# adaliaramon/LambdaGap

Hardware: AMD Instinct MI355X
Metric: boosting iters/sec + AUC, synthetic Higgs-shape 10M×28, 255 bins, 63 leaves (higher is better)
Workload: dtype fp32; 1 GPU; model=gbdt binary, 63 leaves, 255 bins, lr 0.1, global_batch=10000000, seq_len=28, parallelism=dp1, device=AMD GPU (gfx950:sramecc+:xnack-) [frontier engine]

## Files before the change

src/device/device_learner.hip:

```cpp
#include <hip/hip_runtime.h>

#include <algorithm>
#include <chrono>
#include <cmath>
#include <cstdio>
#include <cstdlib>
#include <cstring>
#include <fstream>
#include <map>
#include <memory>
#include <string>
#include <vector>

#include "device/grad_kernels.h"
#include "device/hip_common.h"
#include "device/leaf_kernels.h"
#include "device/metric_kernels.h"
#include "device/linear_kernels.h"
#include "device/runtime_internal.h"
#include "device/frontier.h"
#include "device/policy_scan.h"
#include "device/traverse_kernels.h"
#include "device/sample_kernels.h"
#include "device/engine_plan.h"
#include "device/seq_kernels.h"
#include "device/split_scan.h"
#include "device/tree_kernels.h"
#include "learner/forced_splits.h"
#include "learner/linear_solve.h"
#include "learner/parallel_tree_learner.h"
#include "learner/serial_tree_learner.h"
#include "lgap/common.h"
#include "lgap/device_api.h"
#include "lgap/network.h"
#include "lgap/objective.h"
#include "lgap/rank_math.h"
#include "lgap/metric.h"
#include "lgap/split_math.h"

namespace lgap {
namespace device {
namespace {

const char* KernelOverride(const char* key) {
  static const char* const kKeys[] = {"fhist_threads", "hist_lds_kb", "quant_lds32", "part_iters",
                                      "hist_il",       "nibble",      "quant_hist",  "scan_global",
                                      "scan_wave",     "oob_rows",    "select_merge"};
  constexpr int kNumKeys = static_cast<int>(sizeof(kKeys) / sizeof(kKeys[0]));
  thread_local std::string vals[kNumKeys];
  const char* e = std::getenv("LGAP_KERNEL");
  if (e == nullptr) return nullptr;
  const std::string s(e);
  const char* found = nullptr;
  for (size_t p = 0; p < s.size();) {
    size_t q = s.find(',', p);
    if (q == std::string::npos) q = s.size();
    const std::string item = s.substr(p, q - p);
    p = q + 1;
    if (item.empty()) continue;
    const size_t eq = item.find('=');
    const std::string k = item.substr(0, eq);
    int idx = -1;
    for (int i = 0; i < kNumKeys; ++i) idx = k == kKeys[i] ? i : idx;
    if (idx < 0) Log::Fatal("LGAP_KERNEL: unknown key '%s'", k.c_str());
    if (k == key) {
      vals[idx] = eq == std::string::npos ? "1" : item.substr(eq + 1);
      found = vals[idx].c_str();
    }
  }
  return found;
}


using namespace seq;

template <typename T>
class PinnedBuf {
 public:
  ~PinnedBuf() {
    if (p_) (void)hipHostFree(p_);
  }
  T* Get(size_t n) {
    if (n > n_) {
      if (p_) HIP_CHECK(hipHostFree(p_));
      HIP_CHECK(hipHostMalloc(reinterpret_cast<void**>(&p_), std::max<size_t>(n, 1) * sizeof(T), hipHostMallocDefault));
      n_ = n;
    }
    return p_;
  }

 private:
  T* p_ = nullptr;
  size_t n_ = 0;
};

class DeviceTreeLearner : public TreeLearner {
 public:
  DeviceTreeLearner(const Config* config, const std::string& learner_type, bool routed = false)
      : config_(config), learner_type_(learner_type), routed_(routed) {}

// ... 1555 lines not shown
      if (num_tiles_ > 256) Log::Fatal("frontier histograms: %d LDS tiles (at most 256)", num_tiles_);
    }
    if (ffeature_ || fowner_) {
      std::vector<uint8_t> own(F_, 0);
      std::vector<int> list;
      for (int f : h_own_feat_) {
        if (f >= 0) {
          own[f] = 1;
          list.push_back(f);
        }
      }
      ffowned_.Upload(own, stream_);
      fown_n_ = static_cast<int>(list.size());
      fown_list_.Resize(std::max<size_t>(1, list.size()));
      if (!list.empty()) fown_list_.Upload(list.data(), list.size(), stream_);
      ffpb_.Resize(static_cast<size_t>(P_) * 2 * K);
    }
    if (fowner_) {
      fown_b0_.Upload(h_bin_lo_, stream_);
      const size_t send = static_cast<size_t>(P_) * K * bbin_ * 2;
      if (facc_.size() < send) facc_.Resize(send);
      facc_.Zero(stream_);
      facc_recv_.Resize(static_cast<size_t>(K) * bbin_ * 2);
    }
    if (plan_.bynode_on_device) {
      bool filt = false;
      const std::vector<uint8_t> m = col_sampler_.ByNodeSampleModes(&fbyn_cnt_, &filt);
      fbyn_reset_ = filt ? 1 : 0;
      fbyn_mode_.Resize(m.size());
      fbyn_mode_.Upload(m.data(), m.size(), stream_);
    }
    if (fvoting_) {
      SplitParams sl = MakeArgs().sp;
      sl.min_data_in_leaf = config_->min_data_in_leaf / P_;
      sl.min_sum_hessian_in_leaf = config_->min_sum_hessian_in_leaf / P_;
      fsp_local_.Resize(1);
      fsp_local_.Upload(&sl, 1, stream_);
      flsum_loc_.Resize(C);
      fltot_.Resize(2 * K);
      fltot_.Zero(stream_);
      fvrec_.Resize(static_cast<size_t>(P_) * 2 * K * topk_);
      fvelect_.Resize(2 * K * static_cast<size_t>(topk_ + 1));
      fvrows_.Resize(2 * K * static_cast<size_t>(topk_) * 2 * max_bin_);
    }
    fpart_iters_ = part_iters_;
    fpart_tile_ = kPartThreads * fpart_iters_;
    ftile_cap_ = DivUp(N_, fpart_tile_) + fkmax_ + 1;
    ftile_pub_.Resize(ftile_cap_);
    ftile_pub_.Zero(stream_);
    for (int i = 3; i < kFrontierIdx; ++i) idx_[i].Resize(std::max(N_, 1));
    {
      const int per_cu = std::max(1, FrontierPartitionBlocksPerCU(fpart_iters_));
      fpart_grid_ = std::max(1, std::min(ftile_cap_, per_cu * num_cu_));
    }
    fscan_lds_ = FrontierScanLds(max_bin_, has_cat_ ? max_cat_bin_ : 1);
    FrontierSetLds(FrontierHistLds(), fscan_lds_, use_dp_, width_);
    fspec_cap_ = 0;
    fhist_threads_ = big_tiles_ || (num_tiles_ == 1 && N_ >= 4000000) ? 1024 : 512;
    if (const char* e = KernelOverride("fhist_threads")) fhist_threads_ = std::atoi(e) == 1024 ? 1024 : 512;
    fpolicy_ = 1;
    fspec_alpha_ = 1.0;
    const char* spec_env = std::getenv("LGAP_FRONTIER_SPEC");
    const std::string spec = spec_env != nullptr ? spec_env : "";
    fspec_fixed_ = spec != "adapt";
    if (!spec.empty() && spec != "adapt" && spec != "fixed") {
      char* end = nullptr;
      const double alpha = std::strtod(spec.c_str(), &end);
      if (end == spec.c_str() || *end != '\0') Log::Fatal("LGAP_FRONTIER_SPEC=%s: expected fixed|adapt|<alpha>", spec.c_str());
      fspec_alpha_ = std::max(0.01, std::min(4.0, alpha));
    }
    {
      stune_ = SpecTuner();
      const char* te = std::getenv("LGAP_SPEC_TUNE");
      const bool tune_small = te == nullptr || te[0] != '0';
      stune_.on = !plan_.distributed && (L_ >= 128 || tune_small) && !plan_.raw_cands && fnum_forced_ == 0 &&
                  spec.empty();
      if (L_ < 128 && te == nullptr) stune_.rest = 64;
    }
    if (std::getenv("LGAP_FSTAMPS")) {
      fstamps_.Resize(256 * 4 * kFStampSlots);
      fstamps_.Zero(stream_);
    }
    for (auto& kv : fgraphs_) (void)hipGraphExecDestroy(kv.second);
    fgraphs_.clear();
    if (fcont_) (void)hipGraphExecDestroy(fcont_);
    fcont_ = nullptr;
  }

  FArgs MakeFArgs() const {
    FArgs a;
    std::memset(&a, 0, sizeof(a));
    a.rowbins = rowbins_.get();
    a.colbins = colbins_.get();
    a.gh = gh_.get();
    for (int i = 0; i < kFrontierIdx; ++i) a.idx[i] = idx_[i].get();
    a.N = N_;
    a.stride_dw = tstride_dw_;
    a.width = width_;
    a.num_groups = G_;
    a.TB = TB_;
    a.F = F_;
    a.L = L_;
    a.C = fC_;
    a.kmax = fkmax_;
    a.gstart = gstart_.get();
    a.feat = feat_.get();
// ... 411 lines not shown
    *num_splits = hs->num_splits;
    *num_leaves = hs->num_leaves;
    bynode_draws_ = hs->byn;
    bynode_rng_ = hs->byn_rng;
    if (*num_splits > 0) std::memcpy(hr, fres_host_ + FrontierResultRecOffset(), sizeof(SplitRec) * *num_splits);
    std::memcpy(hrange, fres_host_ + FrontierResultRangeOffset(L_), sizeof(LeafRange) * *num_leaves);
    *hlo = hh->lout0;
    unsigned hbar[4];
    std::memcpy(hbar, hh->bar, sizeof(hbar));
    if (hbar[3] != 0u) {
      static const char* const kinds[kFXKinds] = {"histogram", "split candidates", "root sums", "self-test"};
      Log::Fatal("xGMI exchange (%s) timed out on rank %d after %.0f s: a peer stopped training",
                 kinds[std::min<unsigned>(hbar[3] - 1u, kFXKinds - 1)], rank_, XTimeoutSeconds());
    }
    if (plan_.distributed) {
      std::memcpy(fkused_hist_[fkused_trees_ % 4], hh->kused, sizeof(int) * kFrontierRoundCap);
      ++fkused_trees_;
    }
    if (fstamps_.size() && fstat_trees_ == 3) ReportFrontierStamps(hs->round);
    if (fstamps_.size() && fstat_trees_ % 10 == 0) {
      std::fprintf(stderr, "frontier: %d trees, %.2f rounds/tree, %.2f expansions/tree (%d leaves max), wasted rows %.1f%%, "
                   "alpha %.3f, all-reduced expansion slots/tree %.1f, pipelined rounds/tree %.2f\n", fstat_trees_,
                   static_cast<double>(fstat_rounds_) / fstat_trees_, static_cast<double>(fstat_spec_) / fstat_trees_, L_,
                   100.0 * fstat_waste_ / fstat_trees_, stune_.on ? stune_.lo : fspec_alpha_, fstat_ar_exps_ / fstat_trees_,
                   static_cast<double>(fstat_pipelined_) / fstat_trees_);
    }
  }

  void ReportFrontierStamps(int rounds) {
    std::vector<unsigned long long> h(fstamps_.size());
    fstamps_.Download(h.data(), h.size(), stream_);
    HIP_CHECK(hipStreamSynchronize(stream_));
    static const char* names[4] = {"partition", "hist", "scan", "select"};
    auto at = [&](int r, int k, int i) { return h[(static_cast<size_t>(r) * 4 + k) * kFStampSlots + i]; };
    for (int k = 0; k < 4; ++k) {
      double acc[kFStampSlots] = {0};
      int cnt = 0;
      for (int r = 0; r < std::min(rounds + 1, 256); ++r) {
        const unsigned long long s0 = at(r, k, 0);
        if (!s0) continue;
        ++cnt;
        for (int i = 1; i < kFStampSlots; ++i) {
          const unsigned long long v = at(r, k, i);
          if (v >= s0) acc[i] += (v - s0) * 0.01;
        }
      }
      if (!cnt) continue;
      std::string line;
      for (int i = 1; i < kFStampSlots; ++i) {
        if (acc[i] > 0) line += " t" + std::to_string(i) + "=" + common::FormatG(acc[i] / cnt);
      }
      std::fprintf(stderr, "fstamps %s (%d rounds, us from block-0 start; t7 = last block exit):%s\n", names[k], cnt,
                   line.c_str());
      if (at(0, k, 0)) {
        std::string root;
        for (int i = 1; i < kFStampSlots; ++i) {
          const unsigned long long v = at(0, k, i);
          if (v >= at(0, k, 0) && v) root += " t" + std::to_string(i) + "=" + common::FormatG((v - at(0, k, 0)) * 0.01);
        }
        std::fprintf(stderr, "fstamps %s root round:%s\n", names[k], root.c_str());
      }
    }
    double gap[4] = {0};
    int cnt = 0;
    for (int r = 1; r + 1 < std::min(rounds, 255); ++r) {
      const unsigned long long P = at(r, 0, 0), H = at(r, 1, 0), S = at(r, 2, 0), Q = at(r, 3, 0), P2 = at(r + 1, 0, 0);
      if (!P || !H || !S || !Q || !P2 || !(P < H && H < S && S < Q && Q < P2)) continue;
      gap[0] += (H - P) * 0.01;
      gap[1] += (S - H) * 0.01;
      gap[2] += (Q - S) * 0.01;
      gap[3] += (P2 - Q) * 0.01;
      ++cnt;
    }
    if (cnt) {
      std::fprintf(stderr, "fstamps chain (%d rounds, start to start, us): partition->hist %.2f hist->scan %.2f "
                   "scan->select %.2f select->partition %.2f\n", cnt, gap[0] / cnt, gap[1] / cnt, gap[2] / cnt, gap[3] / cnt);
    }
  }

  void SequentialGrow(int* num_splits, int* num_leaves, SplitRec* hr, LeafRange* hrange, double* hlo) {
    const bool collectives = plan_.owner_scan || plan_.voting;
    const bool use_graph = config_->device_use_graph && (!collectives || (DPGraphEnabled() && !HostStagedDP()));
    if (use_graph) {
      if (graph_exec_ && plan_.distributed && graph_comm_ != ActiveComm()) InvalidateGraph();
      if (!graph_exec_) CaptureGraph();
      HIP_CHECK(hipGraphLaunch(graph_exec_, stream_));
    } else {
      EnqueueTree();
    }
    Ctl* hc2 = pin_ctl_.Get(2);
    HIP_CHECK(hipMemcpyAsync(hc2, ctl_.get(), 2 * sizeof(Ctl), hipMemcpyDeviceToHost, stream_));
    HIP_CHECK(hipMemcpyAsync(hr, rec_.get(), sizeof(SplitRec) * (L_ - 1), hipMemcpyDeviceToHost, stream_));
    HIP_CHECK(hipMemcpyAsync(hrange, range_.get(), sizeof(LeafRange) * L_, hipMemcpyDeviceToHost, stream_));
    HIP_CHECK(hipMemcpyAsync(hlo, lout_.get(), sizeof(double), hipMemcpyDeviceToHost, stream_));
    unsigned* hbar = pin_bar_.Get(4);
    HIP_CHECK(hipMemcpyAsync(hbar, bar_.get(), 4 * sizeof(unsigned), hipMemcpyDeviceToHost, stream_));
    if (collectives && !HostStagedDP()) {
      static const double timeout_s = CommTimeoutSeconds(config_->time_out);
      WatchedStreamSync(stream_, timeout_s, "device tree growth (RCCL histogram reduce-scatter)");
    } else {
      HIP_CHECK(hipStreamSynchronize(stream_));
    }
    if (hbar[2] != 0u) Log::Fatal("k_partition: a wait on published tile counts timed out (blocks not co-resident?)");
    const Ctl* hc = hc2[1].num_splits > hc2[0].num_splits ? &hc2[1] : &hc2[0];
    bynode_draws_ = 1 + 2 * hc->scan_round;
    *num_splits = hc->num_splits;
    *num_leaves = hc->num_leaves;
  }

  std::string DeviceName() const override {
    if (!plan_.owner_scan && !plan_.voting) {
      if (!frontier_) return device_name_;
      if (plan_.mono_inter) return device_name_ + " [frontier engine, intermediate monotone walk + rescans]";
// ... 1749 lines not shown
```

src/device/frontier_kernels.hip:

```cpp
#include <hip/hip_runtime.h>

#include <algorithm>
#include <cstdint>

#include "device/frontier.h"
#include "device/hip_common.h"
#include "device/split_scan.h"
#include "lgap/split_math.h"

namespace lgap {
namespace device {
namespace {

constexpr int kFPartThreads = 256;
constexpr int kFScanThreads = 256;
constexpr int kFSelThreads = 1024;
#ifndef LGAP_FHIST_R
#define LGAP_FHIST_R 16
#endif

__device__ __forceinline__ int FRowAt(const FArgs& a, int buf, int pos) { return buf < 0 ? pos : a.idx[buf][pos]; }

__device__ __forceinline__ uint32_t FColBin(const FArgs& a, int g, int row) {
  const size_t o = static_cast<size_t>(g) * a.N + row;
// ... 1238 lines not shown
      if (lane == 0) {
        key->feature = out->feature;
        key->gain = SafeGain(*out);
        key->threshold = out->threshold;
        key->group = fi.group;
        key->offset = fi.offset;
        key->num_bin = fi.num_bin;
        key->mfb = fi.mfb;
        key->default_bin = fi.default_bin;
        key->missing = fi.missing;
        key->default_left = out->default_left;
        key->is_cat = fi.bin_type != 0 ? 1 : 0;
        key->pad0 = a.cegb_raw && out->feature >= 0 ? out->monotone_type : 0;
      }
      FWaveSync();
      const size_t q = (static_cast<size_t>(e) * 2 + sel) * F + f;
      for (int i = lane; i < kKeyWords + kInfoWords; i += 64) {
        if (i < kKeyWords) {
          reinterpret_cast<uint32_t*>(a.ckey + q)[i] = reinterpret_cast<const uint32_t*>(key)[i];
        } else {
          reinterpret_cast<uint32_t*>(a.cinfo + q)[i - kKeyWords] = reinterpret_cast<const uint32_t*>(out)[i - kKeyWords];
        }
      }
      FWaveSync();
    }
    FWaveSync();
  }
  FStampEnd(a, rnd, kFStampScan);
}


__device__ __forceinline__ void FPublish(unsigned long long* p, unsigned epoch, int v, bool incl) {
  const unsigned long long w = (static_cast<unsigned long long>(epoch) << 32) | (incl ? 0x80000000ull : 0ull) |
                               static_cast<unsigned>(v);
  __hip_atomic_store(p, w, __ATOMIC_RELAXED, __HIP_MEMORY_SCOPE_AGENT);
}

__device__ __forceinline__ bool FGoLeft(const FExp& x, const uint32_t* bits, uint32_t gb) {
  const uint32_t b = DecodeBin(x.offset, x.num_bin, x.mfb, gb);
  if (x.is_cat) {
    const uint32_t wd = b >> 5;
    return wd < static_cast<uint32_t>(kMaxCatWords) && ((bits[wd] >> (b & 31u)) & 1u);
  }
  if ((x.missing == 1 && b == static_cast<uint32_t>(x.default_bin)) ||
      (x.missing == 2 && b == static_cast<uint32_t>(x.num_bin - 1))) {
    return x.default_left != 0;
  }
  return b <= static_cast<uint32_t>(x.thr);
}

constexpr unsigned kLookbackSpins = 2048;

constexpr int kLookbackPer = 4;

struct FLookbackLds {
  int near, nmiss, list[256 * kLookbackPer], val[256 * kLookbackPer], red[4];
};

__device__ int FLookback(const FArgs& a, const FExp& x, const uint32_t* bits, int i, unsigned epoch, FLookbackLds* L) {
  const int t = threadIdx.x;
  const int nt = static_cast<int>(blockDim.x);
  constexpr int kInf = 0x7fffffff;
  int excl = 0;
  for (int hi = i; hi > x.tile0;) {
    const int lo = max(x.tile0, hi - kLookbackPer * nt);
    unsigned long long v[kLookbackPer];
    bool have[kLookbackPer];
    if (t == 0) {
      L->near = kInf;
      L->nmiss = 0;
    }
#pragma unroll
    for (int u = 0; u < kLookbackPer; ++u) {
      const int j = hi - 1 - (u * nt + t);
      v[u] = j >= lo ? __hip_atomic_load(&a.tile_pub[j], __ATOMIC_RELAXED, __HIP_MEMORY_SCOPE_AGENT) : 0ull;
    }
#pragma unroll
    for (int u = 0; u < kLookbackPer; ++u) {
      const int j = hi - 1 - (u * nt + t);
      have[u] = false;
      if (j < lo) continue;
      for (unsigned spins = 0; static_cast<unsigned>(v[u] >> 32) != epoch && spins < kLookbackSpins; ++spins) {
        __builtin_amdgcn_s_sleep(1);
        v[u] = __hip_atomic_load(&a.tile_pub[j], __ATOMIC_RELAXED, __HIP_MEMORY_SCOPE_AGENT);
      }
      have[u] = static_cast<unsigned>(v[u] >> 32) == epoch && !a.part_selfcount;
    }
    __syncthreads();
#pragma unroll
    for (int u = 0; u < kLookbackPer; ++u) {
      const int j = hi - 1 - (u * nt + t);
      if (j >= lo && !have[u]) L->list[atomicAdd(&L->nmiss, 1)] = j;
    }
    __syncthreads();
    const int nm = L->nmiss;
    if (nm > 0) {
      for (int m = 0; m < nm; ++m) {
        const int tile = L->list[m];
        const int p0 = (tile - x.tile0) * a.part_tile, p1 = min(x.count, p0 + a.part_tile);
        int cc = 0;
        for (int p = p0 + t; p < p1; p += nt) {
          const int row = FRowAt(a, x.src_buf, x.start + p);
          cc += FGoLeft(x, bits, FColBin(a, x.group, row)) ? 1 : 0;
        }
        cc = BlockSumInt(cc, L->red);
        if (t == 0) {
          L->val[hi - 1 - tile] = cc;
          FPublish(&a.tile_pub[tile], epoch, cc, false);
        }
      }
      __syncthreads();
#pragma unroll
      for (int u = 0; u < kLookbackPer; ++u) {
        const int j = hi - 1 - (u * nt + t);
        if (j >= lo && !have[u]) {
          v[u] = static_cast<unsigned long long>(static_cast<unsigned>(L->val[u * nt + t]));
          have[u] = true;
        }
      }
    }
#pragma unroll
    for (int u = 0; u < kLookbackPer; ++u) {
      if (have[u] && (v[u] & 0x80000000ull) != 0ull) atomicMin(&L->near, u * nt + t);
    }
    __syncthreads();
    const int near = L->near;
    int c = 0;
#pragma unroll
    for (int u = 0; u < kLookbackPer; ++u) {
      const int j = hi - 1 - (u * nt + t);
      if (j >= lo && u * nt + t <= near) c += static_cast<int>(v[u] & 0x7fffffffull);
    }
    excl += BlockSumInt(c, L->red);
    if (near != kInf) break;
    hi = lo;
  }
  return excl;
}

__device__ void FPostSplit(const FArgs& a, int e, const FExp& x, int lc) {
  const SplitInfo& bi = x.forced >= 0 ? a.fbest[x.parent] : a.best[x.parent];
  const double lsg = bi.left_sum_gradient, lsh = bi.left_sum_hessian;
  const double rsg = bi.right_sum_gradient, rsh = bi.right_sum_hessian;
  const double lo = bi.left_output, ro = bi.right_output;
  const int ilc = bi.left_count, irc = bi.right_count;
  const int8_t mono = bi.monotone_type;
  const int16_t ncat = bi.num_cat_threshold;
  const int feature = bi.feature;
  LeafBounds bl = a.bounds[x.parent];
  const int rc = x.count - lc;
  const int glc = a.distributed ? ilc : lc;
  const int grc = a.distributed ? irc : rc;
  const int l = x.left, r = x.left + 1;
  const int dep = x.depth + 1;
  FNode nl, nr;
  nl.buf = nr.buf = x.dst_buf;
  nl.start = x.start;
  nl.count = lc;
  nl.gcount = glc;
  nr.start = x.start + lc;
  nr.count = rc;
  nr.gcount = grc;
  nl.depth = nr.depth = dep;
  nl.parent = nr.parent = x.parent;
  nl.left = nr.left = -1;
  nl.fidx = x.forced >= 0 ? a.forced[x.forced].left : -1;
  nr.fidx = x.forced >= 0 ? a.forced[x.forced].right : -1;
  a.nodes[l] = nl;
  a.nodes[r] = nr;
  a.lsum[l] = make_double2(lsg, lsh);
  a.lsum[r] = make_double2(rsg, rsh);
  a.lout[l] = lo;
  a.lout[r] = ro;
  LeafBounds br = bl;
  if (a.use_monotone && ncat == 0 && a.mono_inter) {
    if (mono < 0) {
      bl.min = fmax(bl.min, ro);
      br.max = fmin(br.max, lo);
    } else if (mono > 0) {
      bl.max = fmin(bl.max, ro);
      br.min = fmax(br.min, lo);
    }
  } else if (a.use_monotone && ncat == 0) {
    const double mid = (lo + ro) / 2.0f;
    if (mono < 0) {
      bl.min = fmax(bl.min, mid);
      br.max = fmin(br.max, mid);
    } else if (mono > 0) {
      bl.max = fmin(bl.max, mid);
      br.min = fmax(br.min, mid);
    }
  }
  a.bounds[l] = bl;
  a.bounds[r] = br;
  if (a.ic) {
    for (int w = 0; w < a.ic_words; ++w) {
      const unsigned long long icm = a.ic[static_cast<size_t>(x.parent) * a.ic_words + w] &
                                     a.ic_feat[static_cast<size_t>(feature) * a.ic_words + w];
      a.ic[static_cast<size_t>(l) * a.ic_words + w] = icm;
      a.ic[static_cast<size_t>(r) * a.ic_words + w] = icm;
    }
  }
  const int md = a.sp.min_data_in_leaf;
  const bool forced_child = nl.fidx >= 0 || nr.fidx >= 0;
  const bool skip = x.last || (!forced_child && ((a.max_depth > 0 && dep >= a.max_depth) || (grc < md * 2 && glc < md * 2)));
  const bool left_smaller = glc < grc;
  FExp* xo = a.exps + e;
  xo->skip = skip ? 1 : 0;
  xo->smaller = left_smaller ? l : r;
  xo->larger = left_smaller ? r : l;
  xo->h_buf = x.dst_buf;
  xo->h_start = left_smaller ? x.start : x.start + lc;
  xo->h_count = left_smaller ? lc : rc;
}

template <int M>
__device__ __forceinline__ void BlockSumMulti(int* v, int* sh) {
  const int lane = threadIdx.x & 63, w = threadIdx.x >> 6;
#pragma unroll
  for (int m = 0; m < M; ++m) v[m] = WaveSum(v[m]);
  __syncthreads();
  if (lane == 0) {
#pragma unroll
    for (int m = 0; m < M; ++m) sh[m * 4 + w] = v[m];
  }
  __syncthreads();
#pragma unroll
  for (int m = 0; m < M; ++m) v[m] = sh[m * 4] + sh[m * 4 + 1] + sh[m * 4 + 2] + sh[m * 4 + 3];
}

template <int ITERS, int MAXT>
__global__ __launch_bounds__(kFPartThreads) __attribute__((amdgpu_waves_per_eu(ITERS == 8 ? 5 : 1))) void k_f_partition(FArgs a) {
  static_assert(kFPartThreads == 256, "4 waves per block");
  static_assert(MAXT * ITERS <= 32, "left / valid bits of a thread fit one word");
  constexpr int kTile = kFPartThreads * ITERS;
  __shared__ int s_t0[kFrontierKmax + 1];
  __shared__ FExp s_x[kFrontierKmax];
  __shared__ uint32_t s_bits[kFrontierKmax][kMaxCatWords];
  __shared__ int sh[MAXT * 4];
  __shared__ int s_wl[MAXT][ITERS][kFPartThreads / 64];
  __shared__ int s_wv[MAXT][ITERS][kFPartThreads / 64];
  __shared__ FLookbackLds s_lb;
  const FState* stp = a.st;
  if (stp->done) return;
  const int k = stp->k, T = stp->total_tiles;
  const unsigned epoch = stp->epoch;
  const int rnd = stp->round;
  FStamp(a, rnd, kFStampPart, 0);
  const int G = static_cast<int>(gridDim.x);
  const int t = threadIdx.x;
  if (static_cast<int>(blockIdx.x) * MAXT >= T) return;
  constexpr int kXWords = static_cast<int>(sizeof(FExp) / 4);
  for (int i = t; i < k * kXWords; i += blockDim.x) {
    reinterpret_cast<uint32_t*>(s_x)[i] = reinterpret_cast<const uint32_t*>(a.exps)[i];
  }
  for (int i = t; i < k * kMaxCatWords; i += blockDim.x) s_bits[i / kMaxCatWords][i % kMaxCatWords] = a.exp_bits[i];
  __syncthreads();
  if (t <= k) s_t0[t] = t < k ? s_x[t].tile0 : T;
  __syncthreads();
  auto find = [&](int tile) {
    int lo = 0, hi = k - 1;
    while (lo < hi) {
      const int mid = (lo + hi + 1) >> 1;
      if (s_t0[mid] <= tile) lo = mid;
      else hi = mid - 1;
    }
    return lo;
  };
  auto go_left = [&](int e, uint32_t gb) { return FGoLeft(s_x[e], s_bits[e], gb); };
  FStamp(a, rnd, kFStampPart, 1);
  const int lane = t & 63, w = t >> 6;
  const unsigned long long lt_mask = (lane == 0) ? 0ull : (~0ull >> (64 - lane));
  for (int bid = static_cast<int>(blockIdx.x) * MAXT; bid < T; bid += G * MAXT) {
    int ex[MAXT], rows[MAXT][ITERS];
    unsigned lbits = 0u, vbits = 0u;
#pragma unroll
    for (int j = 0; j < MAXT; ++j) {
      const int tile = bid + j;
      ex[j] = tile < T ? find(tile) : -1;
      const int e = ex[j] < 0 ? 0 : ex[j];
      const FExp& x = s_x[e];
      const int pos0 = (tile - x.tile0) * kTile + t;
#pragma unroll
      for (int i = 0; i < ITERS; ++i) {
        const int pos = pos0 + i * kFPartThreads;
        rows[j][i] = (ex[j] >= 0 && pos < x.count) ? FRowAt(a, x.src_buf, x.start + pos) : -1;
      }
    }
    int cnt[MAXT];
    {
      uint32_t gb[MAXT][ITERS];
#pragma unroll
      for (int j = 0; j < MAXT; ++j) {
        const int g = s_x[ex[j] < 0 ? 0 : ex[j]].group;
#pragma unroll
        for (int i = 0; i < ITERS; ++i) gb[j][i] = rows[j][i] >= 0 ? FColBin(a, g, rows[j][i]) : 0u;
      }
#pragma unroll
      for (int j = 0; j < MAXT; ++j) {
        cnt[j] = 0;
#pragma unroll
        for (int i = 0; i < ITERS; ++i) {
          const bool valid = rows[j][i] >= 0;
          const bool left = valid && go_left(ex[j], gb[j][i]);
          vbits |= (valid ? 1u : 0u) << (j * ITERS + i);
          lbits |= (left ? 1u : 0u) << (j * ITERS + i);
          cnt[j] += left ? 1 : 0;
        }
      }
    }
    BlockSumMulti<MAXT>(cnt, sh);
    if (t == 0) {
#pragma unroll
      for (int j = 0; j < MAXT; ++j) {
        if (ex[j] >= 0) FPublish(&a.tile_pub[bid + j], epoch, cnt[j], bid + j == s_x[ex[j]].tile0);
      }
    }
    FStamp(a, rnd, kFStampPart, 2);
    int lb[MAXT];
    lb[0] = ex[0] >= 0 && bid > s_x[ex[0]].tile0 ? FLookback(a, s_x[ex[0]], s_bits[ex[0]], bid, epoch, &s_lb) : 0;
#pragma unroll
    for (int j = 1; j < MAXT; ++j) lb[j] = ex[j] >= 0 && ex[j] == ex[j - 1] ? lb[j - 1] + cnt[j - 1] : 0;
    if (t == 0) {
#pragma unroll
      for (int j = 0; j < MAXT; ++j) {
        if (ex[j] >= 0 && bid + j > s_x[ex[j]].tile0) FPublish(&a.tile_pub[bid + j], epoch, lb[j] + cnt[j], true);
      }
    }
#pragma unroll
    for (int j = 0; j < MAXT; ++j) {
#pragma unroll
      for (int i = 0; i < ITERS; ++i) {
        const unsigned long long ml = __ballot((lbits >> (j * ITERS + i)) & 1u);
        const unsigned long long mv = __ballot((vbits >> (j * ITERS + i)) & 1u);
        if (lane == 0) {
          s_wl[j][i][w] = __popcll(ml);
          s_wv[j][i][w] = __popcll(mv);
        }
      }
    }
    __syncthreads();
#pragma unroll
    for (int j = 0; j < MAXT; ++j) {
      if (ex[j] < 0) continue;
      const int e = ex[j];
      const FExp& x = s_x[e];
      const int tile = bid + j;
      const int tt = tile - x.tile0;
      int lbase = lb[j];
      int rbase = tt * kTile - lbase;
      int* out = a.idx[x.dst_buf] + x.start;
#pragma unroll
      for (int i = 0; i < ITERS; ++i) {
        const bool valid = (vbits >> (j * ITERS + i)) & 1u;
        const bool left = (lbits >> (j * ITERS + i)) & 1u;
        const unsigned long long ml = __ballot(left);
        const unsigned long long mv = __ballot(valid);
        int pl = 0, pv = 0, tl = 0, tv = 0;
#pragma unroll
        for (int q = 0; q < kFPartThreads / 64; ++q) {
          if (q < w) {
            pl += s_wl[j][i][q];
            pv += s_wv[j][i][q];
          }
          tl += s_wl[j][i][q];
          tv += s_wv[j][i][q];
        }
        if (valid) {
          const int rl = pl + __popcll(ml & lt_mask);
          const int rv = pv + __popcll(mv & lt_mask);
          int* dst = left ? out + lbase + rl : out + (x.count - 1 - (rbase + (rv - rl)));
          *dst = rows[j][i];
        }
        lbase += tl;
        rbase += tv - tl;
      }
      if (tt == x.ntiles - 1 && t == 0) FPostSplit(a, e, x, lbase);
    }
    __syncthreads();
  }
  FStamp(a, rnd, kFStampPart, 3);
  FStampEnd(a, rnd, kFStampPart);
}

__device__ __forceinline__ bool FBetter(double ga, int fa, int la, double gb, int fb, int lb) {
  if (ga != gb) return ga > gb;
  if (fa != fb) return fa < fb;
  return la < lb;
}

__device__ __forceinline__ double CegbAdjust(const FArgs& a, const SplitKey& k, int n, int depth, const uint8_t* used,
                                             int node) {
  if (k.feature < 0) return kMinScore;
  double delta = a.cegb_split * n;
  if (a.cegb_coupled != nullptr && !used[k.feature]) delta += a.cegb_coupled[k.feature];
  if (a.cegb_lazy != nullptr) delta += a.cegb_lazy[k.feature] * a.nlazy[static_cast<size_t>(node) * a.F + k.feature];
  double g = k.gain - delta;
  if (k.pad0 != 0) g *= MonotonePenaltyAt(a.monotone_penalty, depth);
  return g;
}

__device__ __forceinline__ void CegbSetBest(const FArgs& a, int c, size_t src, double g) {
  constexpr int kInfoWords = static_cast<int>(sizeof(SplitInfo) / 4);
  constexpr int kKeyWords = static_cast<int>(sizeof(SplitKey) / 4);
  for (int i = 0; i < kInfoWords; ++i) reinterpret_cast<uint32_t*>(a.best + c)[i] = reinterpret_cast<const uint32_t*>(a.ninfo + src)[i];
  for (int i = 0; i < kKeyWords; ++i) reinterpret_cast<uint32_t*>(a.key + c)[i] = reinterpret_cast<const uint32_t*>(a.nkey + src)[i];
  a.best[c].gain = g;
  a.key[c].gain = g;
}

__device__ void FByNodeDraw(const FArgs& a, int c, uint8_t* mask, uint8_t* s_pick, unsigned* rng) {
  const int lane = threadIdx.x & 63, F = a.F;
  const unsigned long long lt = lane == 0 ? 0ull : (~0ull >> (64 - lane));
  int N = 0;
  for (int f0 = 0; f0 < F; f0 += 64) {
    const int f = f0 + lane;
    const bool in = f < F && (!a.byn_reset || a.used_bytree[f]) && FIcAllows(a, c, f);
    N += __popcll(__ballot(in));
  }
  const int K = min(a.byn_cnt, N);
  const int mode = a.byn_mode[N];
  for (int i = lane; i < N; i += 64) s_pick[i] = mode == 1 ? 1 : 0;
  __builtin_amdgcn_fence(__ATOMIC_RELEASE, "workgroup");
  __builtin_amdgcn_wave_barrier();
  __builtin_amdgcn_fence(__ATOMIC_ACQUIRE, "workgroup");
  unsigned x = *rng;
  if (lane == 0 && mode >= 2) {
    if (mode == 2) {
      int got = 0;
      for (int i = 0; i < N; ++i) {
        x = 214013u * x + 2531011u;
        const float r = static_cast<float>(static_cast<int>((x >> 16) & 0x7FFFu)) / 32768.0f;
// ... 2017 lines not shown
    wide ? k_f_select<false, true, false, true><<<1, kFSelThreads, ml, s>>>(a) : k_f_select<false, false, false, true><<<1, kFSelThreads, ml, s>>>(a);
  } else if (a.xg) {
    wide ? k_f_select<false, true, true, false><<<1, kFSelThreads, lds, s>>>(a) : k_f_select<false, false, true, false><<<1, kFSelThreads, lds, s>>>(a);
  } else if (wide) {
    k_f_select<false, true, false, false><<<1, kFSelThreads, lds, s>>>(a);
  } else {
    k_f_select<false, false, false, false><<<1, kFSelThreads, lds, s>>>(a);
  }
  HIP_CHECK(hipGetLastError());
}

void LaunchFrontierVote(const FArgs& a, hipStream_t s) {
  const size_t lds = static_cast<size_t>(a.F) * (sizeof(double) + sizeof(int));
  k_f_vote<<<2 * a.kmax, kVoteThreads, lds, s>>>(a);
  HIP_CHECK(hipGetLastError());
}

void LaunchFrontierElect(const FArgs& a, hipStream_t s) {
  const size_t R = static_cast<size_t>(a.vote_P) * a.vote_k;
  const size_t lds = R * (sizeof(double) + 3 * sizeof(int)) + sizeof(int) * (kVoteThreads / 64) + sizeof(int) * a.vote_k + 16;
  k_f_elect<<<2 * a.kmax, kVoteThreads, lds, s>>>(a);
  HIP_CHECK(hipGetLastError());
}

void LaunchFrontierVoteScan(const FArgs& a, size_t lds, hipStream_t s) {
  k_f_vote_scan<<<2 * a.kmax * a.vote_k, 64, lds, s>>>(a);
  HIP_CHECK(hipGetLastError());
  if (a.xrng != nullptr) {
    k_f_vote_xrng<<<(2 * a.kmax * a.vote_k + 63) / 64, 64, 0, s>>>(a);
    HIP_CHECK(hipGetLastError());
  }
}

void LaunchFrontierPairBest(const FArgs& a, hipStream_t s) {
  k_f_pair_best<<<2 * a.kmax, 64, 0, s>>>(a);
  HIP_CHECK(hipGetLastError());
}

void LaunchFrontierXRoot(const FArgs& a, unsigned* ghmax, hipStream_t s) {
  if (a.xc->P > 64) std::abort();
  k_fx_root<<<1, 64, 0, s>>>(a, ghmax);
  HIP_CHECK(hipGetLastError());
}

void LaunchFrontierXSelfTest(const FArgs& a, int round, int nvals, unsigned* err, hipStream_t s) {
  k_fx_push<<<4, 256, 0, s>>>(a, round, nvals);
  k_fx_check<<<4, 256, 0, s>>>(a, round, nvals, err);
  HIP_CHECK(hipGetLastError());
}


int FrontierPartitionBlocksPerCU(int iters) {
  int per_cu = 0;
  const void* fn = iters == 4    ? reinterpret_cast<const void*>(k_f_partition<4, 1>)
                   : iters == 16 ? reinterpret_cast<const void*>(k_f_partition<16, 1>)
                                 : reinterpret_cast<const void*>(k_f_partition<8, 1>);
  HIP_CHECK(hipOccupancyMaxActiveBlocksPerMultiprocessor(&per_cu, fn, kFPartThreads, 0));
  return per_cu;
}

void LaunchFrontierPartition(const FArgs& a, int iters, int grid, hipStream_t s) {
  if (iters == 4) k_f_partition<4, 1><<<grid, kFPartThreads, 0, s>>>(a);
  else if (iters == 16) k_f_partition<16, 1><<<grid, kFPartThreads, 0, s>>>(a);
  else k_f_partition<8, 1><<<grid, kFPartThreads, 0, s>>>(a);
  HIP_CHECK(hipGetLastError());
}


void FrontierSetLds(size_t hist_lds, size_t scan_lds, bool use_dp, int width) {
  (void)use_dp;
  (void)width;
  if (hist_lds > 64 * 1024) {
    const void* fns[24] = {
        reinterpret_cast<const void*>(k_f_hist<0, 0, 512>),  reinterpret_cast<const void*>(k_f_hist<0, 1, 512>),
        reinterpret_cast<const void*>(k_f_hist<0, 2, 512>),  reinterpret_cast<const void*>(k_f_hist<0, 3, 512>),
        reinterpret_cast<const void*>(k_f_hist<0, 0, 1024>), reinterpret_cast<const void*>(k_f_hist<0, 1, 1024>),
        reinterpret_cast<const void*>(k_f_hist<0, 2, 1024>), reinterpret_cast<const void*>(k_f_hist<0, 3, 1024>),
        reinterpret_cast<const void*>(k_f_hist<1, 3, 512>),  reinterpret_cast<const void*>(k_f_hist<2, 3, 512>),
        reinterpret_cast<const void*>(k_f_hist<1, 3, 1024>), reinterpret_cast<const void*>(k_f_hist<2, 3, 1024>),
        reinterpret_cast<const void*>(k_f_hist<1, 0, 512>),  reinterpret_cast<const void*>(k_f_hist<2, 0, 512>),
        reinterpret_cast<const void*>(k_f_hist<1, 1, 512>),  reinterpret_cast<const void*>(k_f_hist<2, 1, 512>),
        reinterpret_cast<const void*>(k_f_hist<1, 2, 512>),  reinterpret_cast<const void*>(k_f_hist<2, 2, 512>),
        reinterpret_cast<const void*>(k_f_hist<1, 0, 1024>), reinterpret_cast<const void*>(k_f_hist<2, 0, 1024>),
        reinterpret_cast<const void*>(k_f_hist<1, 1, 1024>), reinterpret_cast<const void*>(k_f_hist<2, 1, 1024>),
        reinterpret_cast<const void*>(k_f_hist<1, 2, 1024>), reinterpret_cast<const void*>(k_f_hist<2, 2, 1024>)};
    for (const void* fn : fns) {
      HIP_CHECK(hipFuncSetAttribute(fn, hipFuncAttributeMaxDynamicSharedMemorySize, static_cast<int>(hist_lds)));
    }
  }
  if (scan_lds > 64 * 1024) {
    HIP_CHECK(hipFuncSetAttribute(reinterpret_cast<const void*>(k_f_scan<false>), hipFuncAttributeMaxDynamicSharedMemorySize,
                                  static_cast<int>(scan_lds)));
    HIP_CHECK(hipFuncSetAttribute(reinterpret_cast<const void*>(k_f_scan<true>), hipFuncAttributeMaxDynamicSharedMemorySize,
                                  static_cast<int>(scan_lds)));
  }
  HIP_CHECK(hipFuncSetAttribute(reinterpret_cast<const void*>(k_f_scan_w), hipFuncAttributeMaxDynamicSharedMemorySize,
                                static_cast<int>(std::min<size_t>(150 * 1024, 4 * scan_lds))));
}

}
}
```

Baseline: 389.5 iters/s.

## Restructure frontier partition kernel with chunked tile batches, prefetch and LUT split test

The partition kernel now processes a chunk of four grid-strided tiles per block. It prefetches the next tile's row ids while gathering bins for the current one, and evaluates the split test through a per-wave 256-bit ballot lookup table for narrow bins. Per-tile left counts are accumulated with LDS atomics and published by the last wave, and offsets are computed with a DPP wave scan, which removes the block-wide reductions and the valid-count ballots. The lookback's LDS list shrinks to 64 entries and is processed in rounds. A part_grid override and a fstamps print tweak are also added. The goal is to hide gather latency and cut synchronisation and LDS use, at the cost of more complex control flow and extra LDS for masks.

```diff
diff --git a/src/device/device_learner.hip b/src/device/device_learner.hip
--- a/src/device/device_learner.hip
+++ b/src/device/device_learner.hip
@@ -45,7 +45,7 @@
 const char* KernelOverride(const char* key) {
   static const char* const kKeys[] = {"fhist_threads", "hist_lds_kb", "quant_lds32", "part_iters",
                                       "hist_il",       "nibble",      "quant_hist",  "scan_global",
-                                      "scan_wave",     "oob_rows",    "select_merge"};
+                                      "scan_wave",     "oob_rows",    "select_merge", "part_grid"};
   constexpr int kNumKeys = static_cast<int>(sizeof(kKeys) / sizeof(kKeys[0]));
   thread_local std::string vals[kNumKeys];
   const char* e = std::getenv("LGAP_KERNEL");
@@ -1707,6 +1707,10 @@
     {
       const int per_cu = std::max(1, FrontierPartitionBlocksPerCU(fpart_iters_));
       fpart_grid_ = std::max(1, std::min(ftile_cap_, per_cu * num_cu_));
+      if (const char* e = KernelOverride("part_grid")) {
+        const int v = std::atoi(e);
+        if (v >= 1) fpart_grid_ = std::min(fpart_grid_, v);
+      }
     }
     fscan_lds_ = FrontierScanLds(max_bin_, has_cat_ ? max_cat_bin_ : 1);
     FrontierSetLds(FrontierHistLds(), fscan_lds_, use_dp_, width_);
@@ -2224,13 +2228,14 @@
       }
       std::fprintf(stderr, "fstamps %s (%d rounds, us from block-0 start; t7 = last block exit):%s\n", names[k], cnt,
                    line.c_str());
-      if (at(0, k, 0)) {
+      const int r0 = k == 0 ? 1 : 0;
+      if (at(r0, k, 0)) {
         std::string root;
         for (int i = 1; i < kFStampSlots; ++i) {
-          const unsigned long long v = at(0, k, i);
-          if (v >= at(0, k, 0) && v) root += " t" + std::to_string(i) + "=" + common::FormatG((v - at(0, k, 0)) * 0.01);
+          const unsigned long long v = at(r0, k, i);
+          if (v >= at(r0, k, 0) && v) root += " t" + std::to_string(i) + "=" + common::FormatG((v - at(r0, k, 0)) * 0.01);
         }
-        std::fprintf(stderr, "fstamps %s root round:%s\n", names[k], root.c_str());
+        std::fprintf(stderr, "fstamps %s %s:%s\n", names[k], k == 0 ? "first split" : "root round", root.c_str());
       }
     }
     double gap[4] = {0};
diff --git a/src/device/frontier_kernels.hip b/src/device/frontier_kernels.hip
--- a/src/device/frontier_kernels.hip
+++ b/src/device/frontier_kernels.hip
@@ -1314,9 +1314,10 @@
 constexpr unsigned kLookbackSpins = 2048;
 
 constexpr int kLookbackPer = 4;
+constexpr int kLookbackList = 64;
 
 struct FLookbackLds {
-  int near, nmiss, list[256 * kLookbackPer], val[256 * kLookbackPer], red[4];
+  int near, nmiss, list[kLookbackList], val[kLookbackList], red[4];
 };
 
 __device__ int FLookback(const FArgs& a, const FExp& x, const uint32_t* bits, int i, unsigned epoch, FLookbackLds* L) {
@@ -1348,15 +1349,24 @@
       }
       have[u] = static_cast<unsigned>(v[u] >> 32) == epoch && !a.part_selfcount;
     }
-    __syncthreads();
-#pragma unroll
-    for (int u = 0; u < kLookbackPer; ++u) {
-      const int j = hi - 1 - (u * nt + t);
-      if (j >= lo && !have[u]) L->list[atomicAdd(&L->nmiss, 1)] = j;
-    }
-    __syncthreads();
-    const int nm = L->nmiss;
-    if (nm > 0) {
+    for (;;) {
+      __syncthreads();
+      int slot[kLookbackPer];
+#pragma unroll
+      for (int u = 0; u < kLookbackPer; ++u) {
+        const int j = hi - 1 - (u * nt + t);
+        slot[u] = -1;
+        if (j >= lo && !have[u]) {
+          const int m = atomicAdd(&L->nmiss, 1);
+          if (m < kLookbackList) {
+            L->list[m] = j;
+            slot[u] = m;
+          }
+        }
+      }
+      __syncthreads();
+      const int nm = min(L->nmiss, kLookbackList);
+      if (nm == 0) break;
       for (int m = 0; m < nm; ++m) {
         const int tile = L->list[m];
         const int p0 = (tile - x.tile0) * a.part_tile, p1 = min(x.count, p0 + a.part_tile);
@@ -1367,19 +1377,20 @@
         }
         cc = BlockSumInt(cc, L->red);
         if (t == 0) {
-          L->val[hi - 1 - tile] = cc;
+          L->val[m] = cc;
           FPublish(&a.tile_pub[tile], epoch, cc, false);
         }
       }
       __syncthreads();
 #pragma unroll
       for (int u = 0; u < kLookbackPer; ++u) {
-        const int j = hi - 1 - (u * nt + t);
-        if (j >= lo && !have[u]) {
-          v[u] = static_cast<unsigned long long>(static_cast<unsigned>(L->val[u * nt + t]));
+        if (slot[u] >= 0) {
+          v[u] = static_cast<unsigned long long>(static_cast<unsigned>(L->val[slot[u]]));
           have[u] = true;
         }
       }
+      __syncthreads();
+      if (t == 0) L->nmiss = 0;
     }
 #pragma unroll
     for (int u = 0; u < kLookbackPer; ++u) {
@@ -1476,32 +1487,25 @@
   xo->h_count = left_smaller ? lc : rc;
 }
 
-template <int M>
-__device__ __forceinline__ void BlockSumMulti(int* v, int* sh) {
-  const int lane = threadIdx.x & 63, w = threadIdx.x >> 6;
-#pragma unroll
-  for (int m = 0; m < M; ++m) v[m] = WaveSum(v[m]);
-  __syncthreads();
-  if (lane == 0) {
-#pragma unroll
-    for (int m = 0; m < M; ++m) sh[m * 4 + w] = v[m];
-  }
-  __syncthreads();
-#pragma unroll
-  for (int m = 0; m < M; ++m) v[m] = sh[m * 4] + sh[m * 4 + 1] + sh[m * 4 + 2] + sh[m * 4 + 3];
-}
-
-template <int ITERS, int MAXT>
+constexpr int kFPartChunk = 4;
+
+template <int ITERS>
 __global__ __launch_bounds__(kFPartThreads) __attribute__((amdgpu_waves_per_eu(ITERS == 8 ? 5 : 1))) void k_f_partition(FArgs a) {
   static_assert(kFPartThreads == 256, "4 waves per block");
-  static_assert(MAXT * ITERS <= 32, "left / valid bits of a thread fit one word");
+  static_assert(ITERS <= 32, "the left bits of a thread's rows of one tile fit one word");
   constexpr int kTile = kFPartThreads * ITERS;
+  constexpr int C = kFPartChunk;
+  constexpr int kWaves = kFPartThreads / 64;
+  static_assert(ITERS * kWaves <= 64, "one wave scans a tile's per-(row slot, wave) left counts");
+  constexpr bool kLut = ITERS >= 8;
   __shared__ int s_t0[kFrontierKmax + 1];
   __shared__ FExp s_x[kFrontierKmax];
   __shared__ uint32_t s_bits[kFrontierKmax][kMaxCatWords];
-  __shared__ int sh[MAXT * 4];
-  __shared__ int s_wl[MAXT][ITERS][kFPartThreads / 64];
-  __shared__ int s_wv[MAXT][ITERS][kFPartThreads / 64];
+  __shared__ unsigned s_cnt[C];
+  __shared__ int s_ex[C];
+  __shared__ int s_wl[C][ITERS * kWaves];
+  __shared__ uint32_t s_mask[C][kFPartThreads];
+  __shared__ uint32_t s_lut[kWaves][8];
   __shared__ FLookbackLds s_lb;
   const FState* stp = a.st;
   if (stp->done) return;
@@ -1511,12 +1515,13 @@
   FStamp(a, rnd, kFStampPart, 0);
   const int G = static_cast<int>(gridDim.x);
   const int t = threadIdx.x;
-  if (static_cast<int>(blockIdx.x) * MAXT >= T) return;
+  if (static_cast<int>(blockIdx.x) >= T) return;
   constexpr int kXWords = static_cast<int>(sizeof(FExp) / 4);
   for (int i = t; i < k * kXWords; i += blockDim.x) {
     reinterpret_cast<uint32_t*>(s_x)[i] = reinterpret_cast<const uint32_t*>(a.exps)[i];
   }
   for (int i = t; i < k * kMaxCatWords; i += blockDim.x) s_bits[i / kMaxCatWords][i % kMaxCatWords] = a.exp_bits[i];
+  if (t < C) s_cnt[t] = 0u;
   __syncthreads();
   if (t <= k) s_t0[t] = t < k ? s_x[t].tile0 : T;
   __syncthreads();
@@ -1527,119 +1532,139 @@
       if (s_t0[mid] <= tile) lo = mid;
       else hi = mid - 1;
     }
-    return lo;
+    return __builtin_amdgcn_readfirstlane(lo);
   };
-  auto go_left = [&](int e, uint32_t gb) { return FGoLeft(s_x[e], s_bits[e], gb); };
+  auto load_ids = [&](int e, int tile, int (&r)[ITERS]) {
+    const FExp& x = s_x[e];
+    const int pos0 = (tile - x.tile0) * kTile + t;
+    const int cnt = x.count, start = x.start;
+    const int* src = x.src_buf < 0 ? nullptr : a.idx[x.src_buf] + start;
+#pragma unroll
+    for (int i = 0; i < ITERS; ++i) {
+      const int pos = pos0 + i * kFPartThreads;
+      r[i] = pos < cnt ? (src ? src[pos] : start + pos) : -1;
+    }
+  };
   FStamp(a, rnd, kFStampPart, 1);
   const int lane = t & 63, w = t >> 6;
-  const unsigned long long lt_mask = (lane == 0) ? 0ull : (~0ull >> (64 - lane));
-  for (int bid = static_cast<int>(blockIdx.x) * MAXT; bid < T; bid += G * MAXT) {
-    int ex[MAXT], rows[MAXT][ITERS];
-    unsigned lbits = 0u, vbits = 0u;
-#pragma unroll
-    for (int j = 0; j < MAXT; ++j) {
-      const int tile = bid + j;
-      ex[j] = tile < T ? find(tile) : -1;
-      const int e = ex[j] < 0 ? 0 : ex[j];
+  const bool narrow = a.width == 1;
+  int e_lut = -1;
+  for (int bid = static_cast<int>(blockIdx.x); bid < T; bid += G * C) {
+    int rows0[ITERS], cur[ITERS];
+    int e = find(bid);
+    load_ids(e, bid, cur);
+#pragma unroll 1
+    for (int c = 0; c < C; ++c) {
+      const int tile = bid + c * G;
+      if (tile >= T) break;
       const FExp& x = s_x[e];
-      const int pos0 = (tile - x.tile0) * kTile + t;
+      uint32_t gb[ITERS];
+      if (narrow) {
+        const uint8_t* col = a.colbins + static_cast<size_t>(x.group) * a.N;
+#pragma unroll
+        for (int i = 0; i < ITERS; ++i) gb[i] = col[static_cast<uint32_t>(max(cur[i], 0))];
+      } else {
+        const uint16_t* col = reinterpret_cast<const uint16_t*>(a.colbins) + static_cast<size_t>(x.group) * a.N;
+#pragma unroll
+        for (int i = 0; i < ITERS; ++i) gb[i] = col[static_cast<uint32_t>(max(cur[i], 0))];
+      }
+      int nxt[ITERS];
+      int e_n = e;
+      if (c + 1 < C && tile + G < T) {
+        e_n = find(tile + G);
+        load_ids(e_n, tile + G, nxt);
+      } else {
+#pragma unroll
+        for (int i = 0; i < ITERS; ++i) nxt[i] = -1;
+      }
+      const bool lut = kLut && narrow;
+      if (lut && e != e_lut) {
+        __builtin_amdgcn_fence(__ATOMIC_RELEASE, "wavefront");
+        __builtin_amdgcn_wave_barrier();
+#pragma unroll
+        for (int j = 0; j < 4; ++j) {
+          const unsigned long long bal = __ballot(FGoLeft(x, s_bits[e], static_cast<uint32_t>(lane + 64 * j)));
+          if (lane == 0) {
+            s_lut[w][2 * j] = static_cast<uint32_t>(bal);
+            s_lut[w][2 * j + 1] = static_cast<uint32_t>(bal >> 32);
+          }
+        }
+        __builtin_amdgcn_fence(__ATOMIC_RELEASE, "wavefront");
+        __builtin_amdgcn_wave_barrier();
+        e_lut = e;
+      }
+      int wcnt = 0;
+      uint32_t m = 0u;
 #pragma unroll
       for (int i = 0; i < ITERS; ++i) {
-        const int pos = pos0 + i * kFPartThreads;
-        rows[j][i] = (ex[j] >= 0 && pos < x.count) ? FRowAt(a, x.src_buf, x.start + pos) : -1;
-      }
-    }
-    int cnt[MAXT];
-    {
-      uint32_t gb[MAXT][ITERS];
-#pragma unroll
-      for (int j = 0; j < MAXT; ++j) {
-        const int g = s_x[ex[j] < 0 ? 0 : ex[j]].group;
-#pragma unroll
-        for (int i = 0; i < ITERS; ++i) gb[j][i] = rows[j][i] >= 0 ? FColBin(a, g, rows[j][i]) : 0u;
-      }
-#pragma unroll
-      for (int j = 0; j < MAXT; ++j) {
-        cnt[j] = 0;
-#pragma unroll
-        for (int i = 0; i < ITERS; ++i) {
-          const bool valid = rows[j][i] >= 0;
-          const bool left = valid && go_left(ex[j], gb[j][i]);
-          vbits |= (valid ? 1u : 0u) << (j * ITERS + i);
-          lbits |= (left ? 1u : 0u) << (j * ITERS + i);
-          cnt[j] += left ? 1 : 0;
-        }
-      }
-    }
-    BlockSumMulti<MAXT>(cnt, sh);
-    if (t == 0) {
-#pragma unroll
-      for (int j = 0; j < MAXT; ++j) {
-        if (ex[j] >= 0) FPublish(&a.tile_pub[bid + j], epoch, cnt[j], bid + j == s_x[ex[j]].tile0);
-      }
-    }
+        bool left;
+        if (lut) left = (s_lut[w][(gb[i] >> 5) & 7u] >> (gb[i] & 31u)) & 1u;
+        else left = FGoLeft(x, s_bits[e], gb[i]);
+        left = left && cur[i] >= 0;
+        const int nl = __popcll(__ballot(left));
+        if (lane == 0) s_wl[c][i * kWaves + w] = nl;
+        wcnt += nl;
+        m |= (left ? 1u : 0u) << i;
+      }
+      s_mask[c][t] = m;
+      if (lane == 0) {
+        const unsigned old = atomicAdd(&s_cnt[c], static_cast<unsigned>(wcnt) | (1u << 24));
+        if ((old >> 24) == kWaves - 1) {
+          FPublish(&a.tile_pub[tile], epoch, static_cast<int>(old & 0xffffffu) + wcnt, tile == x.tile0);
+        }
+      }
+      if (t == 0) s_ex[c] = e;
+#pragma unroll
+      for (int i = 0; i < ITERS; ++i) {
+        if (c == 0) rows0[i] = cur[i];
+        cur[i] = nxt[i];
+      }
+      e = e_n;
+    }
+    __syncthreads();
+    for (int c = w; c < C && bid + c * G < T; c += kWaves) {
+      const int v = lane < ITERS * kWaves ? s_wl[c][lane] : 0;
+      const int incl = WaveInclusiveSumDpp(v);
+      if (lane < ITERS * kWaves) s_wl[c][lane] = incl - v;
+    }
+    __syncthreads();
     FStamp(a, rnd, kFStampPart, 2);
-    int lb[MAXT];
-    lb[0] = ex[0] >= 0 && bid > s_x[ex[0]].tile0 ? FLookback(a, s_x[ex[0]], s_bits[ex[0]], bid, epoch, &s_lb) : 0;
-#pragma unroll
-    for (int j = 1; j < MAXT; ++j) lb[j] = ex[j] >= 0 && ex[j] == ex[j - 1] ? lb[j - 1] + cnt[j - 1] : 0;
-    if (t == 0) {
-#pragma unroll
-      for (int j = 0; j < MAXT; ++j) {
-        if (ex[j] >= 0 && bid + j > s_x[ex[j]].tile0) FPublish(&a.tile_pub[bid + j], epoch, lb[j] + cnt[j], true);
-      }
-    }
-#pragma unroll
-    for (int j = 0; j < MAXT; ++j) {
+#pragma unroll 1
+    for (int c = 0; c < C; ++c) {
+      const int tile = bid + c * G;
+      if (tile >= T) break;
+      const int ec = __builtin_amdgcn_readfirstlane(s_ex[c]);
+      const FExp& x = s_x[ec];
+      const int tt = tile - x.tile0;
+      int rows[ITERS];
+      if (c == 0) {
+#pragma unroll
+        for (int i = 0; i < ITERS; ++i) rows[i] = rows0[i];
+      } else {
+        load_ids(ec, tile, rows);
+      }
+      const int lb = tt > 0 ? FLookback(a, x, s_bits[ec], tile, epoch, &s_lb) : 0;
+      const int lend = lb + static_cast<int>(s_cnt[c] & 0xffffffu);
+      if (t == 0 && tt > 0) FPublish(&a.tile_pub[tile], epoch, lend, true);
+      const uint32_t m = s_mask[c][t];
+      int* out = a.idx[x.dst_buf] + x.start;
+      const int last = x.count - 1;
 #pragma unroll
       for (int i = 0; i < ITERS; ++i) {
-        const unsigned long long ml = __ballot((lbits >> (j * ITERS + i)) & 1u);
-        const unsigned long long mv = __ballot((vbits >> (j * ITERS + i)) & 1u);
-        if (lane == 0) {
-          s_wl[j][i][w] = __popcll(ml);
-          s_wv[j][i][w] = __popcll(mv);
-        }
-      }
-    }
-    __syncthreads();
-#pragma unroll
-    for (int j = 0; j < MAXT; ++j) {
-      if (ex[j] < 0) continue;
-      const int e = ex[j];
-      const FExp& x = s_x[e];
-      const int tile = bid + j;
-      const int tt = tile - x.tile0;
-      int lbase = lb[j];
-      int rbase = tt * kTile - lbase;
-      int* out = a.idx[x.dst_buf] + x.start;
-#pragma unroll
-      for (int i = 0; i < ITERS; ++i) {
-        const bool valid = (vbits >> (j * ITERS + i)) & 1u;
-        const bool left = (lbits >> (j * ITERS + i)) & 1u;
+        const bool left = (m >> i) & 1u;
         const unsigned long long ml = __ballot(left);
-        const unsigned long long mv = __ballot(valid);
-        int pl = 0, pv = 0, tl = 0, tv = 0;
-#pragma unroll
-        for (int q = 0; q < kFPartThreads / 64; ++q) {
-          if (q < w) {
-            pl += s_wl[j][i][q];
-            pv += s_wv[j][i][q];
-          }
-          tl += s_wl[j][i][q];
-          tv += s_wv[j][i][q];
-        }
-        if (valid) {
-          const int rl = pl + __popcll(ml & lt_mask);
-          const int rv = pv + __popcll(mv & lt_mask);
-          int* dst = left ? out + lbase + rl : out + (x.count - 1 - (rbase + (rv - rl)));
-          *dst = rows[j][i];
-        }
-        lbase += tl;
-        rbase += tv - tl;
-      }
-      if (tt == x.ntiles - 1 && t == 0) FPostSplit(a, e, x, lbase);
-    }
-    __syncthreads();
+        const int rl = lb + s_wl[c][i * kWaves + w] + static_cast<int>(__builtin_amdgcn_mbcnt_hi(
+                           static_cast<uint32_t>(ml >> 32), __builtin_amdgcn_mbcnt_lo(static_cast<uint32_t>(ml), 0u)));
+        const int p = tt * kTile + i * kFPartThreads + t;
+        if (rows[i] >= 0) out[left ? rl : last - (p - rl)] = rows[i];
+      }
+      if (tt == x.ntiles - 1 && t == 0) FPostSplit(a, ec, x, lend);
+    }
+    if (bid + G * C < T) {
+      __syncthreads();
+      if (t < C) s_cnt[t] = 0u;
+      __syncthreads();
+    }
   }
   FStamp(a, rnd, kFStampPart, 3);
   FStampEnd(a, rnd, kFStampPart);
@@ -3763,17 +3788,17 @@
 
 int FrontierPartitionBlocksPerCU(int iters) {
   int per_cu = 0;
-  const void* fn = iters == 4    ? reinterpret_cast<const void*>(k_f_partition<4, 1>)
-                   : iters == 16 ? reinterpret_cast<const void*>(k_f_partition<16, 1>)
-                                 : reinterpret_cast<const void*>(k_f_partition<8, 1>);
+  const void* fn = iters == 4    ? reinterpret_cast<const void*>(k_f_partition<4>)
+                   : iters == 16 ? reinterpret_cast<const void*>(k_f_partition<16>)
+                                 : reinterpret_cast<const void*>(k_f_partition<8>);
   HIP_CHECK(hipOccupancyMaxActiveBlocksPerMultiprocessor(&per_cu, fn, kFPartThreads, 0));
   return per_cu;
 }
 
 void LaunchFrontierPartition(const FArgs& a, int iters, int grid, hipStream_t s) {
-  if (iters == 4) k_f_partition<4, 1><<<grid, kFPartThreads, 0, s>>>(a);
-  else if (iters == 16) k_f_partition<16, 1><<<grid, kFPartThreads, 0, s>>>(a);
-  else k_f_partition<8, 1><<<grid, kFPartThreads, 0, s>>>(a);
+  if (iters == 4) k_f_partition<4><<<grid, kFPartThreads, 0, s>>>(a);
+  else if (iters == 16) k_f_partition<16><<<grid, kFPartThreads, 0, s>>>(a);
+  else k_f_partition<8><<<grid, kFPartThreads, 0, s>>>(a);
   HIP_CHECK(hipGetLastError());
 }
 
```

Result: faster. 422.2 iters/s (median of 6 runs) (+8.4%).
